# kasvii/GATOR

Measured on AMD Instinct MI355X. Metric: meshes/sec (B=256, J=17) GATOR forward, higher is better.
Workload: dtype f32; 1 GPU; B=256 synthetic Human3.6M 17-joint poses per GPU, GAT+MDR forward fp32; batch_per_gpu=256, global_batch=256, num_joint=17, impl=fused, parallelism=dp1, mode=gather

## Files before the change

### gator_amd/csrc/gat8_forms.h

```cpp
#pragma once
#include "fused_common.h"
#include "fused_state.h"
#include "x3_common.h"
#include "gat8_rows.h"

namespace gator {
namespace {

constexpr int kNT = 5;
enum Gat8UnitId { U_Q, U_K, U_V, U_H0, U_H1, U_PROJ, U_LIN0, U_LIN1, U_BACK, U_FC1, U_FC2, U_COUNT };
struct Gat8Unit { const float* GatBlockPk::*grid; int tiles; };
constexpr Gat8Unit kGat8Units[U_COUNT] = {
    {&GatBlockPk::qkv, 4}, {&GatBlockPk::qkv, 4}, {&GatBlockPk::qkv, 4}, {&GatBlockPk::w0, 4}, {&GatBlockPk::w1, 4}, {&GatBlockPk::proj, 4},
    {&GatBlockPk::lin0, 4}, {&GatBlockPk::lin1, 1}, {&GatBlockPk::back, 4}, {&GatBlockPk::fc1, 16}, {&GatBlockPk::fc2, 16}};
constexpr int gat8_off(int u) {
    int o = 0;
    for (int i = 0; i < u; ++i) o += kGat8Units[i].tiles;
    return o;
}
constexpr int gat8_unit_tile(int u, int w, int i) {
    return u == U_K ? (4 + w) * 4 + i
         : u == U_V ? (8 + w) * 4 + i
         : u == U_LIN1 ? w
         : u == U_BACK ? w * 5 + i
         : u == U_FC1 ? w * 16 + i
         : u == U_FC2 ? w * 16 + 4 * (i & 3) + (i >> 2)
         : w * 4 + i;
}
constexpr int kUseTiles = gat8_off(U_COUNT);
constexpr int kPadTiles = (kNT - kUseTiles % kNT) % kNT;
constexpr int kBlkTiles = kUseTiles + kPadTiles;
constexpr int kWaveTiles = kBlkTiles * kDepth;
constexpr int kStreamTiles = 4 * kWaveTiles + kNT;
constexpr int gat8_slot(int u, int i = 0) { return (gat8_off(u) + i) % kNT; }

template <bool H4, bool H2, bool LB> struct Gat8Stream;

template <> struct Gat8Stream<false, false, false> {
    typedef X3 W;
    typedef X3 O;
    static constexpr int kTileFloats = kTileX3;
    static constexpr bool kByteLo = false, kFoldSmall = false;
    static __device__ __forceinline__ W load(const float* p, int lane) { return x3_load(p, lane); }
    template <bool SWZ = false> static __device__ __forceinline__ O load_opnd(const float* p, int lane) { return x3_load(p, lane); }
    template <bool CL>
    static __device__ __forceinline__ void mma_refill(W& w, const O& b, f32x16& acc, f32x16&, const float* __restrict__ wp, int lane) {
        const bf16x8* q = reinterpret_cast<const bf16x8*>(wp) + lane;
#define GAT8_MM(wpl, bpl, s) acc = CL ? GATOR_MFMA_BF16(b.p[bpl][s], w.p[wpl][s], acc) : GATOR_MFMA_BF16(w.p[wpl][s], b.p[bpl][s], acc)
#pragma unroll
        for (int s = 0; s < 2; ++s) {
            GAT8_MM(2, 0, s);
            __builtin_amdgcn_sched_barrier(0);
            w.p[2][s] = q[(2 * 2 + s) * 64];
            __builtin_amdgcn_sched_barrier(0);
            GAT8_MM(0, 2, s);
            GAT8_MM(1, 1, s);
            GAT8_MM(1, 0, s);
            __builtin_amdgcn_sched_barrier(0);
            w.p[1][s] = q[(1 * 2 + s) * 64];
            __builtin_amdgcn_sched_barrier(0);
            GAT8_MM(0, 1, s);
            GAT8_MM(0, 0, s);
            __builtin_amdgcn_sched_barrier(0);
            w.p[0][s] = q[(0 * 2 + s) * 64];
            __builtin_amdgcn_sched_barrier(0);
        }
#undef GAT8_MM
    }
};

struct Gat8StreamF16 {
    typedef X2 O;
    static constexpr bool kFoldSmall = true;
    template <bool SWZ = false> static __device__ __forceinline__ O load_opnd(const float* p, int lane) { return SWZ ? x2_load_swz(p, lane) : x2_load(p, lane); }
};

template <> struct Gat8Stream<true, false, false> : Gat8StreamF16 {
    typedef H3 W;
    static constexpr int kTileFloats = kTileX3;
    static constexpr bool kByteLo = false;
    static __device__ __forceinline__ W load(const float* p, int lane) { return h3_load(p, lane); }
    template <bool CL>
    static __device__ __forceinline__ void mma_refill(W& w, const O& b, f32x16& acc, f32x16& acs, const float* __restrict__ wp, int lane) {
        const f16x8* q = reinterpret_cast<const f16x8*>(wp) + lane;
#define GAT8_MM(wpl, bpl, s, AC) AC = CL ? GATOR_MFMA_F16(b.p[bpl][s], w.p[wpl][s], AC) : GATOR_MFMA_F16(w.p[wpl][s], b.p[bpl][s], AC)
#pragma unroll
        for (int s = 0; s < 2; ++s) {
            GAT8_MM(0, 1, s, acs);
            GAT8_MM(2, 0, s, acs);
            __builtin_amdgcn_sched_barrier(0);
            w.p[2][s] = q[(2 * 2 + s) * 64];
            __builtin_amdgcn_sched_barrier(0);
            GAT8_MM(1, 0, s, acs);
            __builtin_amdgcn_sched_barrier(0);
            w.p[1][s] = q[(1 * 2 + s) * 64];
            __builtin_amdgcn_sched_barrier(0);
            GAT8_MM(0, 0, s, acc);
            __builtin_amdgcn_sched_barrier(0);
            w.p[0][s] = q[(0 * 2 + s) * 64];
            __builtin_amdgcn_sched_barrier(0);
        }
#undef GAT8_MM
    }
};

template <> struct Gat8Stream<true, true, false> : Gat8StreamF16 {
    typedef G2 W;
    static constexpr int kTileFloats = kTileX3;
    static constexpr bool kByteLo = false;
    static __device__ __forceinline__ W load(const float* p, int lane) {
        const f16x8* q = reinterpret_cast<const f16x8*>(p) + lane;
        W o;
#pragma unroll
        for (int s = 0; s < 2; ++s) o.hi[s] = q[s * 64];
#pragma unroll
        for (int s = 0; s < 2; ++s) o.mid[s] = q[(2 + s) * 64];
        return o;
    }
    template <bool CL>
    static __device__ __forceinline__ void mma_refill(W& w, const O& b, f32x16& acc, f32x16& acs, const float* __restrict__ wp, int lane) {
        const f16x8* q = reinterpret_cast<const f16x8*>(wp) + lane;
#define GAT8_MM(wv, s, AC) AC = CL ? GATOR_MFMA_F16(b.p[0][s], (wv), AC) : GATOR_MFMA_F16((wv), b.p[0][s], AC)
#pragma unroll
        for (int s = 0; s < 2; ++s) {
            GAT8_MM(w.mid[s], s, acs);
            __builtin_amdgcn_sched_barrier(0);
            w.mid[s] = q[(1 * 2 + s) * 64];
            __builtin_amdgcn_sched_barrier(0);
            GAT8_MM(w.hi[s], s, acc);
            __builtin_amdgcn_sched_barrier(0);
            w.hi[s] = q[(0 * 2 + s) * 64];
            __builtin_amdgcn_sched_barrier(0);
        }
#undef GAT8_MM
    }
};

constexpr int kTileH3B = 2 * 512 + 256;
struct H3B { f16x8 p[2][2]; uint4 lo; };
typedef _Float16 f16x2_t __attribute__((ext_vector_type(2)));
__device__ __forceinline__ f16x8 lo_expand(unsigned d0, unsigned d1) {
    const f16x2_t sc = {(_Float16)5.9604644775390625e-08f, (_Float16)5.9604644775390625e-08f};
    union { unsigned u[4]; f16x2_t h[4]; f16x8 v; } o;
    o.u[0] = __builtin_amdgcn_perm(d0, d0, 0x010c000cu);
    o.u[1] = __builtin_amdgcn_perm(d0, d0, 0x030c020cu);
    o.u[2] = __builtin_amdgcn_perm(d1, d1, 0x010c000cu);
    o.u[3] = __builtin_amdgcn_perm(d1, d1, 0x030c020cu);
#pragma unroll
    for (int i = 0; i < 4; ++i) o.h[i] = o.h[i] * sc;
    return o.v;
}
template <> struct Gat8Stream<true, false, true> : Gat8StreamF16 {
    typedef H3B W;
    static constexpr int kTileFloats = kTileH3B;
    static constexpr bool kByteLo = true;
    static __device__ __forceinline__ W load(const float* p, int lane) {
        const f16x8* q = reinterpret_cast<const f16x8*>(p) + lane;
        W o;
#pragma unroll
        for (int pl = 0; pl < 2; ++pl)
#pragma unroll
            for (int s2 = 0; s2 < 2; ++s2) o.p[pl][s2] = q[(pl * 2 + s2) * 64];
        o.lo = reinterpret_cast<const uint4*>(p + 1024)[lane];
        return o;
    }
    template <bool CL>
    static __device__ __forceinline__ void mma_refill(W& w, const O& b, f32x16& acc, f32x16& acs, const float* __restrict__ wp, int lane) {
        const f16x8* q = reinterpret_cast<const f16x8*>(wp) + lane;
#define GAT8_MM(wv, bpl, s, AC) AC = CL ? GATOR_MFMA_F16(b.p[bpl][s], (wv), AC) : GATOR_MFMA_F16((wv), b.p[bpl][s], AC)
#pragma unroll
        for (int s = 0; s < 2; ++s) {
            GAT8_MM(w.p[0][s], 1, s, acs);
            const f16x8 lo = lo_expand(s == 0 ? w.lo.x : w.lo.z, s == 0 ? w.lo.y : w.lo.w);
            GAT8_MM(lo, 0, s, acs);
            __builtin_amdgcn_sched_barrier(0);
            if (s == 1) w.lo = reinterpret_cast<const uint4*>(wp + 1024)[lane];
            __builtin_amdgcn_sched_barrier(0);
            GAT8_MM(w.p[1][s], 0, s, acs);
            __builtin_amdgcn_sched_barrier(0);
            w.p[1][s] = q[(1 * 2 + s) * 64];
            __builtin_amdgcn_sched_barrier(0);
            GAT8_MM(w.p[0][s], 0, s, acc);
            __builtin_amdgcn_sched_barrier(0);
            w.p[0][s] = q[(0 * 2 + s) * 64];
            __builtin_amdgcn_sched_barrier(0);
        }
#undef GAT8_MM
    }
};

template <class F, int S0, bool CL, bool SWZ = false>
__device__ __forceinline__ void unit4(typename F::W (&W)[kNT], const float* __restrict__& wp, typename F::O b, const float* o1, const float* o2,
                                      const float* o3, float* raw, int lane) {
    const float* ops[4] = {o1, o1, o2, o3};
    f32x16 acc = zero16(), acs = zero16();
#pragma unroll
    for (int kb = 0; kb < 4; ++kb) {
        typename F::O bn = b;
        if (kb < 3) bn = F::template load_opnd<SWZ>(ops[kb + 1], lane);
        F::template mma_refill<CL>(W[(S0 + kb) % kNT], b, acc, acs, wp, lane);
        wp += F::kTileFloats;
        b = bn;
    }
    if constexpr (F::kFoldSmall) acc = acc + acs;
    store_block(raw, lane, acc);
}
template <class F, int S0>
__device__ __forceinline__ void unit1(typename F::W (&W)[kNT], const float* __restrict__& wp, const float* o0, float* raw, int lane) {
    f32x16 acc = zero16(), acs = zero16();
    const typename F::O b = F::load_opnd(o0, lane);
    F::template mma_refill<true>(W[S0 % kNT], b, acc, acs, wp, lane);
    wp += F::kTileFloats;
    if constexpr (F::kFoldSmall) acc = acc + acs;
    store_block(raw, lane, acc);
}
template <class F, int S0>
__device__ __forceinline__ void skip_pad(typename F::W (&W)[kNT], const float* __restrict__& wp, int lane) {
#pragma unroll
    for (int i = 0; i < kPadTiles; ++i) {
        W[(S0 + i) % kNT] = F::load(wp, lane);
        wp += F::kTileFloats;
    }
}

}
}
```

### gator_amd/csrc/gat_roles.hip

```cpp
#include "fused_common.h"
#include "fused_state.h"
#include "x3_common.h"
#include "gat8_forms.h"
#include "gat8_rows.h"
#include "gat8_tail.h"

#include <algorithm>
#include <cmath>
#include <cstdlib>
#include <vector>

namespace gator {
namespace {

struct Gat8Blk { const float *back32, *mc, *mdT, *aoffT, *f1b, *vecs; };
struct Gat8Args {
    int B, J;
    const float* pose2d;
    const float *gl0_W, *gl0_b, *gn_w, *gn_b, *gl3_p, *gl3_b, *posT;
    const float *biasT, *m1T, *m2T;
    const float *norm_w, *norm_b;
    const float* wstream;
    Gat8Blk blk[kDepth];
    float* feat;
// ... 30 lines not shown
#else
#define GAT8_BAR(n) __syncthreads()
#define GAT8_SUB(k)
#define GAT8_STAMPS_OUT(n0, n1)
#endif

__device__ __forceinline__ float rsum128(const f32x16 (&x)[4]) {
    float p[4];
#pragma unroll
    for (int q = 0; q < 4; ++q) {
        p[q] = 0.f;
#pragma unroll
        for (int r = 4 * q; r < 4 * q + 4; ++r) p[q] += (x[0][r] + x[1][r]) + (x[2][r] + x[3][r]);
    }
    const float s = (p[0] + p[1]) + (p[2] + p[3]);
    return s + xhalf(s);
}

__device__ __forceinline__ f32x16 ln_own(const float* X, const f32x16& xw, const f32x16& wv, const f32x16& bv, int lane) {
    f32x16 x[4];
#pragma unroll
    for (int kb = 0; kb < 4; ++kb) x[kb] = load_block(X + kb * kTile, lane);
    const float mean = rsum128(x) * (1.0f / 128.0f);
#pragma unroll
    for (int kb = 0; kb < 4; ++kb) { x[kb] = x[kb] - mean; x[kb] = x[kb] * x[kb]; }
    const float rstd = 1.0f / sqrtf(rsum128(x) * (1.0f / 128.0f) + 1e-5f);
    return (xw - mean) * rstd * wv + bv;
}

__device__ __forceinline__ void tile_stats(const f32x16& xw, float* st_w, int lane) {
    float s = 0.f;
#pragma unroll
    for (int q = 0; q < 4; ++q) s += (xw[4 * q] + xw[4 * q + 1]) + (xw[4 * q + 2] + xw[4 * q + 3]);
    s += xhalf(s);
    const float m = s * (1.0f / 32.0f);
    float p[4];
#pragma unroll
    for (int q = 0; q < 4; ++q) {
        p[q] = 0.f;
#pragma unroll
        for (int r = 4 * q; r < 4 * q + 4; ++r) { const float d = xw[r] - m; p[q] += d * d; }
    }
    float m2 = (p[0] + p[1]) + (p[2] + p[3]);
    m2 += xhalf(m2);
    if (lane < 32) { st_w[2 * lane] = m; st_w[2 * lane + 1] = m2; }
}
__device__ __forceinline__ f32x16 ln_stats(const float* ST, const f32x16& xw, const f32x16& wv, const f32x16& bv, int lane) {
    const int tok = lane & 31;
    float m[4], q[4];
#pragma unroll
    for (int i = 0; i < 4; ++i) { m[i] = ST[i * 64 + 2 * tok]; q[i] = ST[i * 64 + 2 * tok + 1]; }
    const float mean = ((m[0] + m[1]) + (m[2] + m[3])) * 0.25f;
    float dev = 0.f;
#pragma unroll
    for (int i = 0; i < 4; ++i) { const float d = m[i] - mean; dev += d * d; }
    const float m2 = ((q[0] + q[1]) + (q[2] + q[3])) + 32.0f * dev;
    const float rstd = 1.0f / sqrtf(m2 * (1.0f / 128.0f) + 1e-5f);
    return (xw - mean) * rstd * wv + bv;
}

__device__ __forceinline__ f32x16 x2_mma_step(const X2& A, const X2& B, int s, f32x16 acc) {
    acc = GATOR_MFMA_F16(A.p[1][s], B.p[0][s], acc);
    acc = GATOR_MFMA_F16(A.p[0][s], B.p[1][s], acc);
    return GATOR_MFMA_F16(A.p[0][s], B.p[0][s], acc);
}

template <bool H4, int LR, bool H2 = false, bool LB = false, bool TAIL = false>
__global__ __launch_bounds__(512, 2) void k_gat8(const Gat8Args a) {
    static_assert(H4 || !TAIL, "the fused tail writes two-plane K / V tiles: four-product forms only");
    using F = Gat8Stream<H4, H2, LB>;
    constexpr int kWF = F::kTileFloats;
    const float inv = H4 ? a.lin_inv : 1.0f;
    const float op16 = ((threadIdx.x & 31) < a.J) ? 16.0f : 0.0f;
    auto st_opnd = [&](float* dst, int lane_, const f32x16& v) {
        if constexpr (H4) x2_store(dst, lane_, x2_split(v * op16)); else x3_store(dst, lane_, x3_split(v));
    };
    auto pick = [&](const float* raw, int lane_, const f32x16& add) {
        if constexpr (H4) return fma16(load_block(raw, lane_), inv, add); else return load_block(raw, lane_) + add;
    };
    extern __shared__ __attribute__((aligned(16))) float lds[];
    float* A = lds + kA;
    float* Bq = lds + kBq;
    float* X = lds + kXo;
    const int b = blockIdx.x, t = threadIdx.x, lane = t & 63, h = lane >> 5, J = a.J;
    const int wave = __builtin_amdgcn_readfirstlane(t >> 6);
    const bool is_prod = wave < 4;
    const int w = wave & 3;
    float* R0w = lds + kR + w * kTile;
    float* R1w = lds + kR + (4 + w) * kTile;
    if constexpr (TAIL) {
        if (a.tl.mdr_ctr)
            for (size_t i = (size_t)b * 512 + t; i < mdr_ctr_words(a.tl.ctr_B); i += (size_t)a.B * 512) a.tl.mdr_ctr[i] = 0u;
    }

    {
        float* hbuf = Bq;
        float* gt = Bq + 2 * kTile;
        float* stat = Bq + 4 * kTile;
        const float* p = a.pose2d + (size_t)b * J * 2;
        for (int e = t; e < 64 * 32; e += 512) {
            const int c = e >> 5, j = e & 31;
            hbuf[e] = j < J ? a.gl0_W[c * 2] * p[j * 2] + a.gl0_W[c * 2 + 1] * p[j * 2 + 1] + a.gl0_b[c] : 0.f;
        }
        __syncthreads();
        if (!is_prod) {
            float s = 0.f;
            for (int e = lane; e < 16 * 32; e += 64) s += ((e & 31) < J) ? hbuf[w * 512 + e] : 0.f;
            for (int o = 32; o > 0; o >>= 1) s += __shfl_xor(s, o);
            const float mean = s / (16.0f * J);
            float q = 0.f;
            for (int e = lane; e < 16 * 32; e += 64) {
                const float d = hbuf[w * 512 + e] - mean;
                q += ((e & 31) < J) ? d * d : 0.f;
            }
            for (int o = 32; o > 0; o >>= 1) q += __shfl_xor(q, o);
            if (lane == 0) { stat[w * 2] = mean; stat[w * 2 + 1] = 1.0f / sqrtf(q / (16.0f * J) + 1e-5f); }
        }
        __syncthreads();
        for (int e = t; e < 2 * kTile; e += 512) {
            const int j4 = e & 3, ln = (e >> 2) & 63, g = (e >> 8) & 3, kb = e >> 10;
            const int tok = ln & 31, c = 32 * kb + 8 * g + 4 * (ln >> 5) + j4;
            gt[e] = tok < J ? gelu_f((hbuf[c * 32 + tok] - stat[(c >> 4) * 2]) * stat[(c >> 4) * 2 + 1] * a.gn_w[c] + a.gn_b[c]) : 0.f;
        }
        __syncthreads();
        if (!is_prod) {
            f32x16 acc = load_chanvec_T(a.gl3_b, 32 * w, h) + load_block(a.posT + (size_t)w * kTile, lane), ac1 = zero16();
            mma2_T(load_wtile(a.gl3_p, w * 2 + 0, lane), load_block(gt, lane), acc, load_wtile(a.gl3_p, w * 2 + 1, lane),
                   load_block(gt + kTile, lane), ac1);
            store_block(X + w * kTile, lane, acc + ac1);
        }
        __syncthreads();
    }

    if (is_prod) {
        typename F::W W[kNT];
        const float* __restrict__ wp = a.wstream + (size_t)w * kWaveTiles * kWF;
#pragma unroll
        for (int s = 0; s < kNT; ++s) { W[s] = F::load(wp, lane); wp += kWF; }
        asm volatile("" ::: "memory");
#ifdef GATOR_DIAG
        unsigned long long* st_lds = reinterpret_cast<unsigned long long*>(lds + kGat8LdsFloats);
        unsigned long long* st_out = (a.stamps && b == 0 && w == 0 && lane == 0) ? st_lds : nullptr;
        if (st_out) for (int i_ = 0; i_ < kDepth * 23 * 2; ++i_) st_lds[i_] = 0;
        unsigned long long st_last = __builtin_amdgcn_s_memtime();
        int bi_ = 0;
#endif
        GAT8_BAR(0);
#pragma unroll 1
        for (int bi = 0; bi < kDepth; ++bi) {
#ifdef GATOR_DIAG
            bi_ = bi;
#endif
            const float *Y0 = A, *Y1 = A + kTileX3, *Y2 = A + 2 * kTileX3, *Y3 = A + 3 * kTileX3;
            typename F::O pre;
            pre = F::load_opnd(Y0, lane);
            unit4<F, gat8_slot(U_Q), false>(W, wp, pre, Y1, Y2, Y3, R0w, lane);
            pre = F::load_opnd(Y0, lane);
            GAT8_BAR(1);
            unit4<F, gat8_slot(U_K), false>(W, wp, pre, Y1, Y2, Y3, R1w, lane);
            pre = F::load_opnd(Y0, lane);
            GAT8_BAR(2);
            unit4<F, gat8_slot(U_V), true>(W, wp, pre, Y1, Y2, Y3, R0w, lane);
            pre = F::load_opnd(Y0, lane);
            GAT8_BAR(3);
            unit4<F, gat8_slot(U_H0), false>(W, wp, pre, Y1, Y2, Y3, R1w, lane);
            pre = F::load_opnd(Y0, lane);
            GAT8_BAR(4);
            unit4<F, gat8_slot(U_H1), true>(W, wp, pre, Y1, Y2, Y3, R0w, lane);
            GAT8_BAR(5);
            pre = F::load_opnd(Bq, lane);
            unit4<F, gat8_slot(U_PROJ), false>(W, wp, pre, Bq + kTileX3, Bq + 2 * kTileX3, Bq + 3 * kTileX3, R1w, lane);
            GAT8_BAR(6);
            GAT8_BAR(7);
            pre = F::load_opnd(Bq + 4 * kTileX3, lane);
            unit4<F, gat8_slot(U_LIN0), true>(W, wp, pre, Bq + 5 * kTileX3, Bq + 6 * kTileX3, Bq + 7 * kTileX3, R0w, lane);
            unit1<F, gat8_slot(U_LIN1)>(W, wp, Bq + (4 + w) * kTileX3, X + w * kTile, lane);
            GAT8_BAR(8);
            GAT8_BAR(9);
            pre = F::load_opnd(Bq + 8 * kTileX3, lane);
            unit4<F, gat8_slot(U_BACK), false>(W, wp, pre, Bq + 9 * kTileX3, Bq + 10 * kTileX3, Bq + 11 * kTileX3, R1w, lane);
            GAT8_BAR(10);
            GAT8_BAR(11);
            GAT8_BAR(12);
            pre = F::load_opnd(Y0, lane);
            unit4<F, gat8_slot(U_FC1, 0), H4>(W, wp, pre, Y1, Y2, Y3, R0w, lane);
            pre = F::load_opnd(Y0, lane);
            GAT8_BAR(13);
            unit4<F, gat8_slot(U_FC1, 4), H4>(W, wp, pre, Y1, Y2, Y3, R1w, lane);
            pre = F::load_opnd(Y0, lane);
            GAT8_BAR(14);
            unit4<F, gat8_slot(U_FC1, 8), H4>(W, wp, pre, Y1, Y2, Y3, R0w, lane);
            pre = F::load_opnd(Y0, lane);
            GAT8_BAR(15);
            unit4<F, gat8_slot(U_FC1, 12), H4>(W, wp, pre, Y1, Y2, Y3, R1w, lane);
            pre = F::template load_opnd<H4>(Bq, lane);
            GAT8_BAR(16);
            unit4<F, gat8_slot(U_FC2, 0), false, H4>(W, wp, pre, Bq + 3 * kTileX3, Bq + 6 * kTileX3, Bq + 9 * kTileX3, R0w, lane);
            pre = F::template load_opnd<H4>(Bq + 1 * kTileX3, lane);
            GAT8_BAR(17);
            unit4<F, gat8_slot(U_FC2, 4), false, H4>(W, wp, pre, Bq + 4 * kTileX3, Bq + 7 * kTileX3, Bq + 10 * kTileX3, R1w, lane);
            pre = F::template load_opnd<H4>(Bq + 2 * kTileX3, lane);
            GAT8_BAR(18);
            unit4<F, gat8_slot(U_FC2, 8), false, H4>(W, wp, pre, Bq + 5 * kTileX3, Bq + 8 * kTileX3, Bq + 11 * kTileX3, R0w, lane);
            pre = F::template load_opnd<H4>(Y0, lane);
            GAT8_BAR(19);
            unit4<F, gat8_slot(U_FC2, 12), false, H4>(W, wp, pre, Y1, Y2, Y3, R1w, lane);
            skip_pad<F, gat8_slot(U_COUNT)>(W, wp, lane);
            GAT8_BAR(20);
            if constexpr (TAIL) {
                if (bi + 1 == kDepth) {
                    if (a.tl.jkv) {
                        const Gat8Tail& tl = a.tl;
                        if (t < VJ_TOTAL / 4) joint_stage_vecs(tl, lds + kTVJ, t);
                        for (int e = t; e < 2 * kTile / 4; e += 256)
                            reinterpret_cast<f32x4*>(lds + kTPosj)[e] = reinterpret_cast<const f32x4*>(tl.posj_T)[e];
                    }
                }
            }
            GAT8_BAR(21);
            GAT8_BAR(22);
        }
        GAT8_STAMPS_OUT(0, kDepth * 23 * 2);
        if constexpr (TAIL) gat8_tail<LR, false>(a.tl, a.pose2d, lds, b, J, w, lane);
        return;
    }

    const int tok = lane & 31;
    const HidAddr hid = hid_addr(lane);
#ifdef GATOR_DIAG
    if (a.dbg & 1) {
        for (int n = 0; n < 1 + 22 * kDepth; ++n) __syncthreads();
        return;
    }
    if (a.dbg & 16) {
        __syncthreads();
        for (int bi = 0; bi < kDepth; ++bi)
            for (int n = 1; n <= 22; ++n) {
                if ((n == 2 || n == 19) && bi + 1 < kDepth && a.pf_loads > 0) {
                    const char* wsrc = reinterpret_cast<const char*>(a.wstream + ((size_t)w * kWaveTiles + (size_t)(bi + 1) * kBlkTiles) * kWF);
                    const int share = a.pf_loads * 8192, first = ((b >> 3) % a.pf_n) * share, lim = kBlkTiles * kWF * 4 - 128;
                    const int i0 = n == 2 ? 0 : (a.pf_loads + 1) / 2, i1 = n == 2 ? (a.pf_loads + 1) / 2 : a.pf_loads;
                    for (int i = i0; i < i1; ++i)
                        glds<4>(reinterpret_cast<const float*>(wsrc + min(first + i * 8192 + lane * 128, lim)), lds + kDummy + w * 256);
                }
                __syncthreads();
            }
        return;
    }
    unsigned long long* st_lds = reinterpret_cast<unsigned long long*>(lds + kGat8LdsFloats);
    unsigned long long* st_out = (a.stamps && b == 0 && w == 0 && lane == 0) ? st_lds + (size_t)kDepth * 23 * 2 : nullptr;
    if (st_out) for (int i_ = 0; i_ < kDepth * 23 * 2 + kDepth * 8; ++i_) st_out[i_] = 0;
    unsigned long long st_last = __builtin_amdgcn_s_memtime();
    int bi_ = 0;
#endif
    f32x16 xw = load_block(X + w * kTile, lane);
    {
        const float* vec = a.blk[0].vecs;
        const f32x16 y = ln_own(X, xw, load_chanvec_T(vec, V_N1W + 32 * w, h), load_chanvec_T(vec, V_N1B + 32 * w, h), lane);
        st_opnd(A + w * kTileX3, lane, y);
    }
    GAT8_BAR(0);
#pragma unroll 1
    for (int bi = 0; bi < kDepth; ++bi) {
#ifdef GATOR_DIAG
        bi_ = bi;
#endif
        const Gat8Blk& kb = a.blk[bi];
        const float* vec = kb.vecs;
        const bool warm = bi + 1 < kDepth && a.pf_loads > 0;
        const float* dummy = lds + kDummy + w * 256;
        const Gat8Blk& nx = a.blk[bi + 1 < kDepth ? bi + 1 : bi];
        auto warm_weights = [&](int i0, int i1) {
            const char* wsrc = reinterpret_cast<const char*>(a.wstream + ((size_t)w * kWaveTiles + (size_t)(bi + 1) * kBlkTiles) * kWF);
            const int share = a.pf_loads * 8192, first = ((b >> 3) % a.pf_n) * share, lim = kBlkTiles * kWF * 4 - 128;
            for (int i = i0; i < i1; ++i)
                glds<4>(reinterpret_cast<const float*>(wsrc + min(first + i * 8192 + lane * 128, lim)), dummy);
        };
        const f32x16 bq = load_chanvec_T(vec, V_QKVB + 32 * w, h), bk = load_chanvec_T(vec, V_QKVB + 128 + 32 * w, h);
        const float vb = vec[V_QKVB + 256 + 32 * w + tok];
        const f32x16 ba = load_block(a.biasT + (size_t)(2 * w) * kTile, lane), bb = load_block(a.biasT + (size_t)(2 * w + 1) * kTile, lane);
        GAT8_BAR(1);
        const f32x16 q = pick(R0w, lane, bq);
        X2 qx;
        if constexpr (H4) qx = x2_split(q * op16);
        if (warm) warm_weights(0, (a.pf_loads + 1) / 2);
        if constexpr (TAIL) {
            if (bi + 1 == kDepth && a.tl.warm_n > 0) {
                const int idx = ((b >> 3) % a.tl.warm_n) * 4 + w, parts = a.tl.warm_n * 4;
                auto touch = [&](const float* base, int bytes) {
                    const int share = ((bytes / parts + 127) / 128) * 128;
                    for (int off = lane * 128; off < share; off += 8192)
                        glds<4>(reinterpret_cast<const float*>(reinterpret_cast<const char*>(base) + min(idx * share + off, bytes - 128)), dummy);
                };
                touch(a.tl.lifter_w, 3 * J * kC * J * 4);
                if (a.tl.jkv) {
                    touch(a.tl.jf_h3, 8 * kTileX3 * 4);
#pragma unroll 1
                    for (int li = 0; li < 3; ++li) touch(a.tl.j_wk_h3[li], 8 * kTileX3 * 4);
                }
            }
        }
        GAT8_BAR(2);
        f32x16 sa = zero16(), sb = zero16();
        {
            const f32x16 k = pick(R1w, lane, bk);
            float sscale = 0.25f;
            if constexpr (H4) {
                const X2 kx = x2_split(k * op16);
                sa = GATOR_MFMA_F16(kx.p[1][0], qx.p[0][0], sa);
                sb = GATOR_MFMA_F16(kx.p[1][1], qx.p[0][1], sb);
                sa = GATOR_MFMA_F16(kx.p[0][0], qx.p[1][0], sa);
                sb = GATOR_MFMA_F16(kx.p[0][1], qx.p[1][1], sb);
                sa = GATOR_MFMA_F16(kx.p[0][0], qx.p[0][0], sa);
                sb = GATOR_MFMA_F16(kx.p[0][1], qx.p[0][1], sb);
                sscale = 0.25f / 256.0f;
            } else {
#pragma unroll
                for (int r = 0; r < 8; ++r) {
                    sa = GATOR_MFMA(k[r], q[r], sa);
                    sb = GATOR_MFMA(k[r + 8], q[r + 8], sb);
                }
            }
#pragma unroll
            for (int r = 0; r < 16; ++r) {
                if (r < LR) {
                    const bool ok = kap(r) + 4 * h < J;
                    sa[r] = ok ? (sa[r] * sscale + ba[r]) * kLog2e : -1e30f;
                    sb[r] = ok ? (sb[r] * sscale + bb[r]) * kLog2e : -1e30f;
                } else {
                    sa[r] = 0.f;
                    sb[r] = 0.f;
                }
            }
            float ma = sa[0], mb = sb[0], la, lb;
            {
#pragma unroll
                for (int r = 1; r < LR; ++r) { ma = fmaxf(ma, sa[r]); mb = fmaxf(mb, sb[r]); }
                ma = fmaxf(ma, xhalf(ma));
                mb = fmaxf(mb, xhalf(mb));
#pragma unroll
                for (int r = 0; r < LR; ++r) {
                    sa[r] = __builtin_amdgcn_exp2f(sa[r] - ma);
                    sb[r] = __builtin_amdgcn_exp2f(sb[r] - mb);
                }
                float pa[4], pb[4];
#pragma unroll
                for (int q4 = 0; q4 < 4; ++q4) {
                    pa[q4] = tree4<LR>(q4, [&](int r) { return sa[r]; });
                    pb[q4] = tree4<LR>(q4, [&](int r) { return sb[r]; });
                }
                la = LR > 12 ? (pa[0] + pa[1]) + (pa[2] + pa[3]) : LR > 8 ? (pa[0] + pa[1]) + pa[2] : pa[0] + pa[1];
                lb = LR > 12 ? (pb[0] + pb[1]) + (pb[2] + pb[3]) : LR > 8 ? (pb[0] + pb[1]) + pb[2] : pb[0] + pb[1];
            }
            la += xhalf(la);
            lb += xhalf(lb);
            const float ia = 1.0f / la, ib = 1.0f / lb;
#pragma unroll
            for (int r = 0; r < LR; ++r) { sa[r] = sa[r] * ia; sb[r] = sb[r] * ib; }
        }
// ... 159 lines not shown
        hidden(R1w, A + w * kTileX3, fb1);
        const f32x16 bfc2 = load_chanvec_T(vec, V_FC2B + 32 * w, h);
        GAT8_BAR(17);
        f32x16 c01 = pick(R0w, lane, bfc2);
        GAT8_BAR(18);
        c01 = pick(R1w, lane, c01);
        if (warm) warm_weights((a.pf_loads + 1) / 2, a.pf_loads);
        if (warm) {
            const int l32 = lane & 31;
            glds<4>(h == 0 ? nx.mdT + (size_t)w * kTile + l32 * 32 : nx.mc + (size_t)w * kTile + l32 * 32, dummy);
            if (w == 0) glds<4>(nx.vecs + lane * 32, dummy);
            if (w == 1) glds<4>(h == 0 ? nx.aoffT + l32 * 32 : nx.f1b + l32 * 32, dummy);
            glds<4>(nx.back32 + (size_t)(w * 5 + 4) * kTile + (lane & 15) * 32, dummy);
        }
        GAT8_BAR(19);
        f32x16 c23 = load_block(R0w, lane);
        if constexpr (H4) c23 = c23 * inv;
        const bool last = bi + 1 == kDepth;
        const float* nvec = last ? a.norm_w : a.blk[bi + 1 < kDepth ? bi + 1 : bi].vecs + V_N1W;
        const float* nvecb = last ? a.norm_b : a.blk[bi + 1 < kDepth ? bi + 1 : bi].vecs + V_N1B;
        const f32x16 nw = load_chanvec_T(nvec, 32 * w, h), nb = load_chanvec_T(nvecb, 32 * w, h);
        GAT8_BAR(20);
        c23 = pick(R1w, lane, c23);
        xw += c01 + c23;
        tile_stats(xw, lds + kStat + w * 64, lane);
        if (a.blk_tap && tok < J) {
            store_row_block(a.blk_tap + (((size_t)bi * a.tapB + b) * J + tok) * kC + 32 * w, h, xw);
        }
        GAT8_BAR(21);
        {
            f32x16 y = ln_stats(lds + kStat, xw, nw, nb, lane);
            if (!last) {
                st_opnd(A + w * kTileX3, lane, y);
            } else {
                gelu_pairs<8>(y);
                if (tok < J) store_row_block(a.feat + ((size_t)b * J + tok) * kC + 32 * w, h, y);
                if constexpr (TAIL) {
                    if (tok >= J) y = zero16();
                    store_block(X + w * kTile, lane, y);
                }
            }
        }
        GAT8_BAR(22);
    }
    GAT8_STAMPS_OUT(kDepth * 23 * 2, 2 * kDepth * 23 * 2 + kDepth * 8);
    if constexpr (TAIL) gat8_tail<LR, true>(a.tl, a.pose2d, lds, b, J, w, lane);
}

}

constexpr size_t kGat8Lds = (size_t)(kGat8LdsFloats + kDiagLdsFloats) * sizeof(float);

using Gat8Kernel = void (*)(const Gat8Args);
struct Gat8Entry { Gat8Form form; Gat8Kernel kernel; int tile_floats; bool byte_lo; };
template <bool H4, int LR, bool H2 = false, bool LB = false, bool TAIL = false>
constexpr Gat8Entry gat8_entry() {
    using F = Gat8Stream<H4, H2, LB>;
    return {{H4, LR, H2, LB, TAIL}, k_gat8<H4, LR, H2, LB, TAIL>, F::kTileFloats, F::kByteLo};
}
const Gat8Entry kGat8Kernels[] = {
    gat8_entry<false, 16>(), gat8_entry<true, 10>(), gat8_entry<true, 12>(), gat8_entry<true, 10, true>(), gat8_entry<true, 12, true>(),
    gat8_entry<true, 10, false, true>(), gat8_entry<true, 12, false, true>(), gat8_entry<true, 10, true, false, true>(),
    gat8_entry<true, 12, true, false, true>(), gat8_entry<true, 10, false, true, true>(), gat8_entry<true, 12, false, true, true>()};

int gat8_prepare_device() {
    for (const auto& e : kGat8Kernels)
        GATOR_HIP_CHECK(hipFuncSetAttribute((const void*)e.kernel, hipFuncAttributeMaxDynamicSharedMemorySize, (int)kGat8Lds));
    return GATOR_OK;
}

#ifdef GATOR_DIAG
constexpr int kGat8Stamps = 2 * kDepth * 23 * 2 + kDepth * 8;
struct Gat8Diag { DevBuf<unsigned long long> stamps, tstamps; };

static int gat8_diag_setup(const FusedState* f, bool tail, Gat8Args& a, Gat8Diag& d) {
    a.stamps = nullptr;
    a.dbg = f->opt.gat8_dbg;
    a.tl.tstamps = nullptr;
    if (!f->opt.gat_stamps) return GATOR_OK;
    GATOR_TRY(d.stamps.alloc(kGat8Stamps * sizeof(unsigned long long)));
    a.stamps = d.stamps.get();
    GATOR_HIP_CHECK(hipMemset(a.stamps, 0, kGat8Stamps * sizeof(unsigned long long)));
    if (tail) {
        GATOR_TRY(d.tstamps.alloc(64 * sizeof(unsigned long long)));
        a.tl.tstamps = d.tstamps.get();
        GATOR_HIP_CHECK(hipMemset(a.tl.tstamps, 0, 64 * sizeof(unsigned long long)));
    }
    return GATOR_OK;
}

static int gat8_diag_report(Gat8Diag& d, int B) {
    if (d.tstamps) {
        unsigned long long ts[64];
        GATOR_HIP_CHECK(hipMemcpy(ts, d.tstamps, sizeof(ts), hipMemcpyDeviceToHost));
        d.tstamps.reset();
        fprintf(stderr, "[k_gat8 tail stamps, one workgroup, B=%d] s_memtime cycles since wave 0 entered: entry | loads issued + joint-token MFMAs | lifter done | at barrier | past barrier | jf + LN done | job 1 | job 2\n", B);
        for (int v = 0; v < 8; ++v) {
            fprintf(stderr, "  wave %d:", v);
            for (int k = 0; k < 8; ++k) fprintf(stderr, " %6lld", ts[v * 8 + k] ? (long long)(ts[v * 8 + k] - ts[0]) : -1LL);
            fprintf(stderr, "\n");
        }
    }
    if (d.stamps) {
        std::vector<unsigned long long> hs(kGat8Stamps);
        GATOR_HIP_CHECK(hipMemcpy(hs.data(), d.stamps, kGat8Stamps * sizeof(unsigned long long), hipMemcpyDeviceToHost));
        d.stamps.reset();
        double tot[2] = {0, 0};
        fprintf(stderr, "[k_gat8 stamps, wg0, B=%d] cycles per step, mean of blocks 1-5: step | product work wait | helper work wait\n", B);
        for (int n = 0; n < 23; ++n) {
            double v[4] = {0, 0, 0, 0};
            for (int role = 0; role < 2; ++role)
                for (int bi = 1; bi < kDepth; ++bi)
                    for (int k = 0; k < 2; ++k) v[role * 2 + k] += (double)hs[(((size_t)role * kDepth + bi) * 23 + n) * 2 + k] / (kDepth - 1);
            fprintf(stderr, "  %2d | %7.0f %7.0f | %7.0f %7.0f\n", n, v[0], v[1], v[2], v[3]);
            tot[0] += v[0] + v[1]; tot[1] += v[2] + v[3];
        }
        fprintf(stderr, "  per block: product %.0f, helper %.0f cycles\n", tot[0], tot[1]);
        fprintf(stderr, "  helper sub-stamps of step 15 (block 1), cycles since the barrier:");
        for (int k = 0; k < 8; ++k) fprintf(stderr, " %llu", hs[(size_t)2 * kDepth * 23 * 2 + 1 * 8 + k]);
        fprintf(stderr, "\n");
    }
    return GATOR_OK;
}
#endif

int launch_gat8(gator_ctx* c, FusedState* f, FusedWs& ws, const ForwardPlan& p, const float* pose2d, int B_total, float* pose3d, void* stream) {
    const Gat8Entry* e = nullptr;
    for (const auto& k : kGat8Kernels)
        if (k.form == p.gat8) e = &k;
    if (!e) return fail(GATOR_EINVAL, "k_gat8: no such form");
    const int row0 = p.n_tiled, B = B_total - row0;
    const size_t o = (size_t)row0 * c->J;
    Gat8Args a;
    const Weights& w = c->w;
    a.B = B; a.J = c->J; a.pose2d = pose2d + o * 2;
    a.gl0_W = w.gl0_W; a.gl0_b = w.gl0_b; a.gn_w = w.gn_w; a.gn_b = w.gn_b; a.gl3_p = f->g_gl3; a.gl3_b = w.gl3_b; a.posT = f->g_posT;
    a.biasT = f->g_biasT; a.m1T = f->g_m1T; a.m2T = f->g_m2T;
    a.norm_w = w.norm_w; a.norm_b = w.norm_b;
    a.wstream = e->byte_lo ? f->g8stream_b.get() : f->g8stream.get();
    for (int i = 0; i < kDepth; ++i) {
        const GatBlockPk& b = f->gblk[i];
        a.blk[i] = Gat8Blk{b.back, b.mc, b.mdT, b.aoffT, b.f1b, f->g_vecs + (size_t)i * V_TOTAL};
    }
    a.feat = ws.feat + o * kC;
    a.tl = Gat8Tail{};
    const bool tail = p.gat8.tail;
    if (tail) {
        Gat8Tail& tl = a.tl;
        tl.lifter_w = w.lifter_w; tl.lifter_b = w.lifter_b; tl.x_out = pose3d + o * 3; tl.jkv = ws.jkv + (size_t)row0 * 12 * kTile;
        if (p.ctr_zero == CtrZero::GAT8_TAIL) { tl.mdr_ctr = ws.mdr_ctr; tl.ctr_B = B_total; }
        tl.jf5 = f->jfeat5; tl.jf_h3 = f->jf128_h3; tl.jf_b = w.jfeat_b; tl.posj_T = f->posj_T;
        auto h3_of = [&](const float* t) { return f->wxbuf + (size_t)(t - f->lay[0].wq) / kTile * kTileX3; };
        for (int i = 0; i < 3; ++i) { tl.j_n1w[i] = w.lay[i].n1w; tl.j_n1b[i] = w.lay[i].n1b; tl.j_wk_h3[i] = h3_of(f->lay[i].wk); tl.j_wv_h3[i] = h3_of(f->lay[i].wv); }
        tl.jf_inv = std::ldexp(1.0f, -(4 + f->jf128_wshift));
        tl.kv_inv = std::ldexp(1.0f, -(4 + f->mdr_wshift));
    }
    a.blk_tap = nullptr;
    a.tapB = B;
    if (c->block_taps) {
        GATOR_TRY(gat_ensure_blk_tap(c, f, B_total));
        a.blk_tap = f->blk_tap + (size_t)row0 * c->J * kC; a.tapB = B_total;
    }
    a.pf_n = std::min(32, (B + 7) / 8);
    a.pf_loads = (kBlkTiles * e->tile_floats * 4 / a.pf_n + 8191) / 8192;
    if (a.pf_loads > 6) a.pf_loads = 0;
    a.tl.warm_n = (tail && a.pf_n >= 8) ? a.pf_n : 0;
    a.lin_inv = std::ldexp(1.0f, -(4 + f->gat8_wshift));
#ifdef GATOR_DIAG
    Gat8Diag diag;
    GATOR_TRY(gat8_diag_setup(f, tail, a, diag));
#endif
    e->kernel<<<B, 512, kGat8Lds, (hipStream_t)stream>>>(a);
    GATOR_HIP_CHECK(hipGetLastError());
#ifdef GATOR_DIAG
    GATOR_TRY(gat8_diag_report(diag, B));
#endif
    return GATOR_OK;
}

}
```

Before: 437,700 meshes/sec.

## Start the next GEMM unit's first tiles before the block barrier

Splits each four-tile matmul unit into a head and a rest so that, for steps whose operands are already published, the first one to four MFMA tiles of the next unit run before the workgroup barrier rather than after it. Per-format tables pick how many tiles start early, and compile-time checks confirm that a head start only reads operand tiles published at an earlier step. The aim is to hide barrier wait time behind matrix work. In exchange, more accumulator state stays live across the barrier, which may raise register pressure. A host-side check that the wk and wv tiles are contiguous is also added.

Result: no change. 435,500 meshes/sec (-0.5%).

```diff
diff --git a/gator_amd/csrc/gat8_forms.h b/gator_amd/csrc/gat8_forms.h
--- a/gator_amd/csrc/gat8_forms.h
+++ b/gator_amd/csrc/gat8_forms.h
@@ -9,10 +9,11 @@
 
 constexpr int kNT = 5;
 enum Gat8UnitId { U_Q, U_K, U_V, U_H0, U_H1, U_PROJ, U_LIN0, U_LIN1, U_BACK, U_FC1, U_FC2, U_COUNT };
-struct Gat8Unit { const float* GatBlockPk::*grid; int tiles; };
+struct Gat8Unit { const float* GatBlockPk::*grid; int tiles; int step; int pub; int pub_inc; };
 constexpr Gat8Unit kGat8Units[U_COUNT] = {
-    {&GatBlockPk::qkv, 4}, {&GatBlockPk::qkv, 4}, {&GatBlockPk::qkv, 4}, {&GatBlockPk::w0, 4}, {&GatBlockPk::w1, 4}, {&GatBlockPk::proj, 4},
-    {&GatBlockPk::lin0, 4}, {&GatBlockPk::lin1, 1}, {&GatBlockPk::back, 4}, {&GatBlockPk::fc1, 16}, {&GatBlockPk::fc2, 16}};
+    {&GatBlockPk::qkv, 4, 1, 0, 0}, {&GatBlockPk::qkv, 4, 2, 0, 0}, {&GatBlockPk::qkv, 4, 3, 0, 0}, {&GatBlockPk::w0, 4, 4, 0, 0},
+    {&GatBlockPk::w1, 4, 5, 0, 0}, {&GatBlockPk::proj, 4, 6, 5, 0}, {&GatBlockPk::lin0, 4, 8, 7, 0}, {&GatBlockPk::lin1, 1, 8, 7, 0},
+    {&GatBlockPk::back, 4, 10, 9, 0}, {&GatBlockPk::fc1, 16, 13, 12, 0}, {&GatBlockPk::fc2, 16, 17, 14, 1}};
 constexpr int gat8_off(int u) {
     int o = 0;
     for (int i = 0; i < u; ++i) o += kGat8Units[i].tiles;
@@ -34,6 +35,43 @@
 constexpr int kStreamTiles = 4 * kWaveTiles + kNT;
 constexpr int gat8_slot(int u, int i = 0) { return (gat8_off(u) + i) % kNT; }
 
+#ifndef GATOR_GAT8_AHEAD
+#define GATOR_GAT8_AHEAD 1
+#endif
+struct Gat8Ahead { int t[23]; };
+constexpr Gat8Ahead kGat8AheadNone = {{0, 0, 0, 0, 0, 0, 0, 0, 0, 0, 0, 0, 0, 0, 0, 0, 0, 0, 0, 0, 0, 0, 0}};
+constexpr Gat8Ahead kGat8AheadX3   = {{0, 0, 0, 0, 0, 0, 0, 0, 0, 0, 0, 0, 0, 0, 1, 2, 3, 4, 2, 2, 0, 0, 0}};
+constexpr Gat8Ahead kGat8AheadH3   = {{0, 0, 0, 4, 0, 0, 0, 0, 0, 0, 0, 0, 0, 0, 1, 2, 3, 4, 2, 2, 0, 0, 0}};
+constexpr Gat8Ahead kGat8AheadG2   = {{0, 0, 0, 4, 0, 0, 0, 0, 0, 0, 0, 0, 0, 0, 1, 2, 3, 4, 1, 2, 0, 0, 0}};
+constexpr int gat8_step_pub(int n) {
+    for (int u = 0; u < U_COUNT; ++u)
+        for (int s = 0; 4 * s + 4 <= kGat8Units[u].tiles; ++s)
+            if (kGat8Units[u].step + s == n) return kGat8Units[u].pub + s * kGat8Units[u].pub_inc;
+    return -1;
+}
+constexpr bool gat8_ahead_legal(const Gat8Ahead& a) {
+    if (a.t[0] != 0 || a.t[22] != 0) return false;
+    for (int n = 1; n < 22; ++n) {
+        if (a.t[n] == 0) continue;
+        if (a.t[n] < 0 || a.t[n] > 4) return false;
+        const int pub = gat8_step_pub(n + 1);
+        if (pub < 0 || pub > n - 1) return false;
+    }
+    return true;
+}
+static_assert(gat8_ahead_legal(kGat8AheadNone) && gat8_ahead_legal(kGat8AheadX3) && gat8_ahead_legal(kGat8AheadH3) && gat8_ahead_legal(kGat8AheadG2),
+              "k_gat8: a head start reads operand tiles that are not published yet");
+constexpr bool gat8_ahead_rule_ok() {
+    for (int n = 1; n < 22; ++n) {
+        Gat8Ahead a = kGat8AheadNone;
+        a.t[n] = 1;
+        const bool want = (n >= 1 && n <= 4) || (n >= 13 && n <= 19);
+        if (gat8_ahead_legal(a) != want) return false;
+    }
+    return true;
+}
+static_assert(gat8_ahead_rule_ok(), "k_gat8: the legality rule of the head start does not match the block's steps");
+
 template <bool H4, bool H2, bool LB> struct Gat8Stream;
 
 template <> struct Gat8Stream<false, false, false> {
@@ -41,6 +79,7 @@
     typedef X3 O;
     static constexpr int kTileFloats = kTileX3;
     static constexpr bool kByteLo = false, kFoldSmall = false;
+    static constexpr Gat8Ahead kAhead = kGat8AheadX3;
     static __device__ __forceinline__ W load(const float* p, int lane) { return x3_load(p, lane); }
     template <bool SWZ = false> static __device__ __forceinline__ O load_opnd(const float* p, int lane) { return x3_load(p, lane); }
     template <bool CL>
@@ -79,6 +118,7 @@
     typedef H3 W;
     static constexpr int kTileFloats = kTileX3;
     static constexpr bool kByteLo = false;
+    static constexpr Gat8Ahead kAhead = kGat8AheadH3;
     static __device__ __forceinline__ W load(const float* p, int lane) { return h3_load(p, lane); }
     template <bool CL>
     static __device__ __forceinline__ void mma_refill(W& w, const O& b, f32x16& acc, f32x16& acs, const float* __restrict__ wp, int lane) {
@@ -108,6 +148,7 @@
     typedef G2 W;
     static constexpr int kTileFloats = kTileX3;
     static constexpr bool kByteLo = false;
+    static constexpr Gat8Ahead kAhead = kGat8AheadG2;
     static __device__ __forceinline__ W load(const float* p, int lane) {
         const f16x8* q = reinterpret_cast<const f16x8*>(p) + lane;
         W o;
@@ -154,6 +195,7 @@
     typedef H3B W;
     static constexpr int kTileFloats = kTileH3B;
     static constexpr bool kByteLo = true;
+    static constexpr Gat8Ahead kAhead = kGat8AheadH3;
     static __device__ __forceinline__ W load(const float* p, int lane) {
         const f16x8* q = reinterpret_cast<const f16x8*>(p) + lane;
         W o;
@@ -189,22 +231,37 @@
     }
 };
 
-template <class F, int S0, bool CL, bool SWZ = false>
-__device__ __forceinline__ void unit4(typename F::W (&W)[kNT], const float* __restrict__& wp, typename F::O b, const float* o1, const float* o2,
-                                      const float* o3, float* raw, int lane) {
+template <class F> struct Gat8Carry { f32x16 acc, acs; typename F::O b; };
+template <class F, int S0, bool CL, bool SWZ, int N0, int N1>
+__device__ __forceinline__ void unit4_tiles(typename F::W (&W)[kNT], const float* __restrict__& wp, Gat8Carry<F>& c, const float* o1, const float* o2,
+                                            const float* o3, int lane) {
     const float* ops[4] = {o1, o1, o2, o3};
-    f32x16 acc = zero16(), acs = zero16();
-#pragma unroll
-    for (int kb = 0; kb < 4; ++kb) {
-        typename F::O bn = b;
+#pragma unroll
+    for (int kb = N0; kb < N1; ++kb) {
+        typename F::O bn = c.b;
         if (kb < 3) bn = F::template load_opnd<SWZ>(ops[kb + 1], lane);
-        F::template mma_refill<CL>(W[(S0 + kb) % kNT], b, acc, acs, wp, lane);
+        F::template mma_refill<CL>(W[(S0 + kb) % kNT], c.b, c.acc, c.acs, wp, lane);
         wp += F::kTileFloats;
-        b = bn;
-    }
-    if constexpr (F::kFoldSmall) acc = acc + acs;
-    store_block(raw, lane, acc);
-}
+        c.b = bn;
+    }
+}
+template <class F, int S0, bool CL, bool SWZ, int N>
+__device__ __forceinline__ void unit4_head(typename F::W (&W)[kNT], const float* __restrict__& wp, Gat8Carry<F>& c, const float* o0, const float* o1,
+                                           const float* o2, const float* o3, int lane) {
+    static_assert(N >= 0 && N <= 4, "a unit has four tiles");
+    c.acc = zero16();
+    c.acs = zero16();
+    c.b = F::template load_opnd<SWZ>(o0, lane);
+    unit4_tiles<F, S0, CL, SWZ, 0, N>(W, wp, c, o1, o2, o3, lane);
+}
+template <class F, int S0, bool CL, bool SWZ, int N>
+__device__ __forceinline__ void unit4_rest(typename F::W (&W)[kNT], const float* __restrict__& wp, Gat8Carry<F>& c, const float* o1, const float* o2,
+                                           const float* o3, float* raw, int lane) {
+    unit4_tiles<F, S0, CL, SWZ, N, 4>(W, wp, c, o1, o2, o3, lane);
+    if constexpr (F::kFoldSmall) c.acc = c.acc + c.acs;
+    store_block(raw, lane, c.acc);
+}
+template <class F> constexpr int gat8_ahead(int n) { return GATOR_GAT8_AHEAD ? F::kAhead.t[n] : 0; }
 template <class F, int S0>
 __device__ __forceinline__ void unit1(typename F::W (&W)[kNT], const float* __restrict__& wp, const float* o0, float* raw, int lane) {
     f32x16 acc = zero16(), acs = zero16();
diff --git a/gator_amd/csrc/gat_roles.hip b/gator_amd/csrc/gat_roles.hip
--- a/gator_amd/csrc/gat_roles.hip
+++ b/gator_amd/csrc/gat_roles.hip
@@ -206,59 +206,63 @@
             bi_ = bi;
 #endif
             const float *Y0 = A, *Y1 = A + kTileX3, *Y2 = A + 2 * kTileX3, *Y3 = A + 3 * kTileX3;
-            typename F::O pre;
-            pre = F::load_opnd(Y0, lane);
-            unit4<F, gat8_slot(U_Q), false>(W, wp, pre, Y1, Y2, Y3, R0w, lane);
-            pre = F::load_opnd(Y0, lane);
+            Gat8Carry<F> c;
+#define GAT8_HEAD(n, slot, CL, SWZ, o0, o1, o2, o3) unit4_head<F, slot, CL, SWZ, gat8_ahead<F>(n)>(W, wp, c, o0, o1, o2, o3, lane)
+#define GAT8_REST(n, slot, CL, SWZ, o1, o2, o3, raw) unit4_rest<F, slot, CL, SWZ, gat8_ahead<F>(n)>(W, wp, c, o1, o2, o3, raw, lane)
+            GAT8_HEAD(0, gat8_slot(U_Q), false, false, Y0, Y1, Y2, Y3);
+            GAT8_REST(0, gat8_slot(U_Q), false, false, Y1, Y2, Y3, R0w);
+            GAT8_HEAD(1, gat8_slot(U_K), false, false, Y0, Y1, Y2, Y3);
             GAT8_BAR(1);
-            unit4<F, gat8_slot(U_K), false>(W, wp, pre, Y1, Y2, Y3, R1w, lane);
-            pre = F::load_opnd(Y0, lane);
+            GAT8_REST(1, gat8_slot(U_K), false, false, Y1, Y2, Y3, R1w);
+            GAT8_HEAD(2, gat8_slot(U_V), true, false, Y0, Y1, Y2, Y3);
             GAT8_BAR(2);
-            unit4<F, gat8_slot(U_V), true>(W, wp, pre, Y1, Y2, Y3, R0w, lane);
-            pre = F::load_opnd(Y0, lane);
+            GAT8_REST(2, gat8_slot(U_V), true, false, Y1, Y2, Y3, R0w);
+            GAT8_HEAD(3, gat8_slot(U_H0), false, false, Y0, Y1, Y2, Y3);
             GAT8_BAR(3);
-            unit4<F, gat8_slot(U_H0), false>(W, wp, pre, Y1, Y2, Y3, R1w, lane);
-            pre = F::load_opnd(Y0, lane);
+            GAT8_REST(3, gat8_slot(U_H0), false, false, Y1, Y2, Y3, R1w);
+            GAT8_HEAD(4, gat8_slot(U_H1), true, false, Y0, Y1, Y2, Y3);
             GAT8_BAR(4);
-            unit4<F, gat8_slot(U_H1), true>(W, wp, pre, Y1, Y2, Y3, R0w, lane);
+            GAT8_REST(4, gat8_slot(U_H1), true, false, Y1, Y2, Y3, R0w);
             GAT8_BAR(5);
-            pre = F::load_opnd(Bq, lane);
-            unit4<F, gat8_slot(U_PROJ), false>(W, wp, pre, Bq + kTileX3, Bq + 2 * kTileX3, Bq + 3 * kTileX3, R1w, lane);
+            GAT8_HEAD(0, gat8_slot(U_PROJ), false, false, Bq, Bq + kTileX3, Bq + 2 * kTileX3, Bq + 3 * kTileX3);
+            GAT8_REST(0, gat8_slot(U_PROJ), false, false, Bq + kTileX3, Bq + 2 * kTileX3, Bq + 3 * kTileX3, R1w);
             GAT8_BAR(6);
             GAT8_BAR(7);
-            pre = F::load_opnd(Bq + 4 * kTileX3, lane);
-            unit4<F, gat8_slot(U_LIN0), true>(W, wp, pre, Bq + 5 * kTileX3, Bq + 6 * kTileX3, Bq + 7 * kTileX3, R0w, lane);
+            GAT8_HEAD(0, gat8_slot(U_LIN0), true, false, Bq + 4 * kTileX3, Bq + 5 * kTileX3, Bq + 6 * kTileX3, Bq + 7 * kTileX3);
+            GAT8_REST(0, gat8_slot(U_LIN0), true, false, Bq + 5 * kTileX3, Bq + 6 * kTileX3, Bq + 7 * kTileX3, R0w);
             unit1<F, gat8_slot(U_LIN1)>(W, wp, Bq + (4 + w) * kTileX3, X + w * kTile, lane);
             GAT8_BAR(8);
             GAT8_BAR(9);
-            pre = F::load_opnd(Bq + 8 * kTileX3, lane);
-            unit4<F, gat8_slot(U_BACK), false>(W, wp, pre, Bq + 9 * kTileX3, Bq + 10 * kTileX3, Bq + 11 * kTileX3, R1w, lane);
+            GAT8_HEAD(0, gat8_slot(U_BACK), false, false, Bq + 8 * kTileX3, Bq + 9 * kTileX3, Bq + 10 * kTileX3, Bq + 11 * kTileX3);
+            GAT8_REST(0, gat8_slot(U_BACK), false, false, Bq + 9 * kTileX3, Bq + 10 * kTileX3, Bq + 11 * kTileX3, R1w);
             GAT8_BAR(10);
             GAT8_BAR(11);
             GAT8_BAR(12);
-            pre = F::load_opnd(Y0, lane);
-            unit4<F, gat8_slot(U_FC1, 0), H4>(W, wp, pre, Y1, Y2, Y3, R0w, lane);
-            pre = F::load_opnd(Y0, lane);
+            GAT8_HEAD(0, gat8_slot(U_FC1, 0), H4, false, Y0, Y1, Y2, Y3);
+            GAT8_REST(0, gat8_slot(U_FC1, 0), H4, false, Y1, Y2, Y3, R0w);
+            GAT8_HEAD(13, gat8_slot(U_FC1, 4), H4, false, Y0, Y1, Y2, Y3);
             GAT8_BAR(13);
-            unit4<F, gat8_slot(U_FC1, 4), H4>(W, wp, pre, Y1, Y2, Y3, R1w, lane);
-            pre = F::load_opnd(Y0, lane);
+            GAT8_REST(13, gat8_slot(U_FC1, 4), H4, false, Y1, Y2, Y3, R1w);
+            GAT8_HEAD(14, gat8_slot(U_FC1, 8), H4, false, Y0, Y1, Y2, Y3);
             GAT8_BAR(14);
-            unit4<F, gat8_slot(U_FC1, 8), H4>(W, wp, pre, Y1, Y2, Y3, R0w, lane);
-            pre = F::load_opnd(Y0, lane);
+            GAT8_REST(14, gat8_slot(U_FC1, 8), H4, false, Y1, Y2, Y3, R0w);
+            GAT8_HEAD(15, gat8_slot(U_FC1, 12), H4, false, Y0, Y1, Y2, Y3);
             GAT8_BAR(15);
-            unit4<F, gat8_slot(U_FC1, 12), H4>(W, wp, pre, Y1, Y2, Y3, R1w, lane);
-            pre = F::template load_opnd<H4>(Bq, lane);
+            GAT8_REST(15, gat8_slot(U_FC1, 12), H4, false, Y1, Y2, Y3, R1w);
+            GAT8_HEAD(16, gat8_slot(U_FC2, 0), false, H4, Bq, Bq + 3 * kTileX3, Bq + 6 * kTileX3, Bq + 9 * kTileX3);
             GAT8_BAR(16);
-            unit4<F, gat8_slot(U_FC2, 0), false, H4>(W, wp, pre, Bq + 3 * kTileX3, Bq + 6 * kTileX3, Bq + 9 * kTileX3, R0w, lane);
-            pre = F::template load_opnd<H4>(Bq + 1 * kTileX3, lane);
+            GAT8_REST(16, gat8_slot(U_FC2, 0), false, H4, Bq + 3 * kTileX3, Bq + 6 * kTileX3, Bq + 9 * kTileX3, R0w);
+            GAT8_HEAD(17, gat8_slot(U_FC2, 4), false, H4, Bq + 1 * kTileX3, Bq + 4 * kTileX3, Bq + 7 * kTileX3, Bq + 10 * kTileX3);
             GAT8_BAR(17);
-            unit4<F, gat8_slot(U_FC2, 4), false, H4>(W, wp, pre, Bq + 4 * kTileX3, Bq + 7 * kTileX3, Bq + 10 * kTileX3, R1w, lane);
-            pre = F::template load_opnd<H4>(Bq + 2 * kTileX3, lane);
+            GAT8_REST(17, gat8_slot(U_FC2, 4), false, H4, Bq + 4 * kTileX3, Bq + 7 * kTileX3, Bq + 10 * kTileX3, R1w);
+            GAT8_HEAD(18, gat8_slot(U_FC2, 8), false, H4, Bq + 2 * kTileX3, Bq + 5 * kTileX3, Bq + 8 * kTileX3, Bq + 11 * kTileX3);
             GAT8_BAR(18);
-            unit4<F, gat8_slot(U_FC2, 8), false, H4>(W, wp, pre, Bq + 5 * kTileX3, Bq + 8 * kTileX3, Bq + 11 * kTileX3, R0w, lane);
-            pre = F::template load_opnd<H4>(Y0, lane);
+            GAT8_REST(18, gat8_slot(U_FC2, 8), false, H4, Bq + 5 * kTileX3, Bq + 8 * kTileX3, Bq + 11 * kTileX3, R0w);
+            GAT8_HEAD(19, gat8_slot(U_FC2, 12), false, H4, Y0, Y1, Y2, Y3);
             GAT8_BAR(19);
-            unit4<F, gat8_slot(U_FC2, 12), false, H4>(W, wp, pre, Y1, Y2, Y3, R1w, lane);
+            GAT8_REST(19, gat8_slot(U_FC2, 12), false, H4, Y1, Y2, Y3, R1w);
+#undef GAT8_HEAD
+#undef GAT8_REST
             skip_pad<F, gat8_slot(U_COUNT)>(W, wp, lane);
             GAT8_BAR(20);
             if constexpr (TAIL) {
@@ -724,6 +728,8 @@
         tl.jf5 = f->jfeat5; tl.jf_h3 = f->jf128_h3; tl.jf_b = w.jfeat_b; tl.posj_T = f->posj_T;
         auto h3_of = [&](const float* t) { return f->wxbuf + (size_t)(t - f->lay[0].wq) / kTile * kTileX3; };
         for (int i = 0; i < 3; ++i) { tl.j_n1w[i] = w.lay[i].n1w; tl.j_n1b[i] = w.lay[i].n1b; tl.j_wk_h3[i] = h3_of(f->lay[i].wk); tl.j_wv_h3[i] = h3_of(f->lay[i].wv); }
+        for (int i = 0; i < 3; ++i)
+            if (tl.j_wv_h3[i] != tl.j_wk_h3[i] + 4 * kTileX3) return fail(GATOR_EINVAL, "k_gat8: a layer's wk and wv tiles are not contiguous in the H3 image");
         tl.jf_inv = std::ldexp(1.0f, -(4 + f->jf128_wshift));
         tl.kv_inv = std::ldexp(1.0f, -(4 + f->mdr_wshift));
     }
```
